# ay-lab/fithic

Measured on AMD Instinct MI355X. Metric: contact-pairs/sec through spline+p-value+BH pass (5 kb cis, whole node), higher is better.
Workload: dtype f64

## Files before the change

### fithic_amd/csrc/fhx_ctx.hpp

```cpp
#pragma once
#include <hip/hip_runtime.h>

#include <atomic>
#include <functional>
#include <chrono>
#include <thread>
#include <memory>
#include <sys/stat.h>
#include <unistd.h>
#include <deque>
#include <mutex>
#include <map>
#include <condition_variable>
#include <algorithm>
#include <climits>
#include <cstddef>
#include <cmath>
#include <cstdio>
#include <cstdlib>
#include <cstring>
#include <string>
#include <vector>

#include "../../include/fithic_mi355x.h"
#include "fhx_bdtrc.hpp"
#include "fhx_devmem.hpp"
#include "fhx_host.hpp"
#include "fhx_io_internal.hpp"
#include "fhx_scan.hpp"

namespace fhx {

__device__ __forceinline__ long long wave_sum_i64(long long v) {
#pragma unroll
    for (int off = 32; off > 0; off >>= 1) v += __shfl_down(v, off, 64);
    return v;
}
__device__ __forceinline__ int wave_max_i32(int v) {
#pragma unroll
    for (int off = 32; off > 0; off >>= 1) v = max(v, __shfl_down(v, off, 64));
    return v;
}

__device__ __forceinline__ unsigned int wave_incl_sum_u32(unsigned int v) {
    v += (unsigned int)__builtin_amdgcn_update_dpp(0, (int)v, 0x111, 0xf, 0xf, false);
    v += (unsigned int)__builtin_amdgcn_update_dpp(0, (int)v, 0x112, 0xf, 0xf, false);
    v += (unsigned int)__builtin_amdgcn_update_dpp(0, (int)v, 0x114, 0xf, 0xf, false);
    v += (unsigned int)__builtin_amdgcn_update_dpp(0, (int)v, 0x118, 0xf, 0xf, false);
    v += (unsigned int)__builtin_amdgcn_update_dpp(0, (int)v, 0x142, 0xa, 0xf, false);
    v += (unsigned int)__builtin_amdgcn_update_dpp(0, (int)v, 0x143, 0xc, 0xf, false);
    return v;
}

struct ChrGrid {
    int32_t base;
    int32_t off;
    int32_t nslots;
    int32_t pad;
};

struct K1Sums {
    long long inter_count, inter_sum, intra_all_count, intra_all_sum, in_range_count, in_range_sum, n_skipped;
    int max_count, pad;
};

struct K2Params {
    const int32_t* loc1;
    const int32_t* loc2;
    const int32_t* count;
    const double* slot_bias;
    bool no_bias;
    const double* prior_lut;
    int lut_len;
    dev::BinomTables intra, inter;
    double inter_chr_prob;
    double outlier_thres;
    int lo_idx, hi_idx;
    int mode;
    int64_t n;
    double* p;
    unsigned long long* top_hist;
    uint8_t* outlier;
    int nonfixed;
    const int32_t* slot_mid;
    const double* table_x;
    const double* table_y;
    int n_table;
    double min_x, max_x;
    long long dist_low, dist_up;
    double total_intra, total_inter;
};

constexpr int K2_THREADS = 256;

constexpr int K2_QUEUES = dev::BC_COUNT - 1;

struct QEntry {
    unsigned int row;
    int count;
    double prior;
};

constexpr int K2_MAX_SHARDS = 2048;

struct QSpan {
    QEntry* base;
    long long cap_s;
    int dir;
    int n_shards;
    const unsigned long long* count;
};
__device__ __forceinline__ QEntry* qentry(const QSpan& q, int shard, long long j) {
    return q.base + (long long)shard * q.cap_s + (long long)q.dir * j;
}

struct K2Queues {
    QSpan q[K2_QUEUES + 1];
    unsigned long long* count;
    unsigned int* heavy_hist;
};

constexpr int K2H_BUCKETS = 2048;
constexpr int K2H_BLOCKS = 1024;
__device__ __forceinline__ int k2h_bucket(int signed_count);

struct CutoffToHost {
    volatile unsigned long long* words = nullptr;
    unsigned long long ticket = 0;
    unsigned int* done = nullptr;
    unsigned long long* zero_me = nullptr;
};

constexpr int K3_DENSE_PERCENT = 35;
constexpr int K2_COUNTER_WORDS = 8;
constexpr int FDR_BUCKETS = 51;

struct DeviceWords {
    unsigned long long bh_kept;
    unsigned long long bh_cutoff;
    unsigned long long bh_below;
    unsigned long long array_kept;
    unsigned long long array_cutoff;
    unsigned long long sort_n;
    unsigned long long run_total;
    unsigned long long nf_keys;
    unsigned long long outliers_added;
    unsigned long long first_dup;
    unsigned long long memo_overflow;
    alignas(128) unsigned long long k2_redo;
    unsigned long long k2_next[K2_COUNTER_WORDS - 1];
    alignas(128) unsigned long long k3_dense;
    unsigned long long k3_sparse;
    alignas(128) unsigned long long fdr_buckets[FDR_BUCKETS];
};
static_assert(offsetof(DeviceWords, k2_next) == offsetof(DeviceWords, k2_redo) + sizeof(unsigned long long) &&
                  sizeof(DeviceWords::k2_next) == (K2_COUNTER_WORDS - 1) * sizeof(unsigned long long),
              "k2_closed zeroes K2_COUNTER_WORDS words starting at k2_redo");
static_assert(K2_COUNTER_WORDS >= 2 + K2_QUEUES, "k2_next holds k2h_heavy's word and one per class queue");
static_assert(sizeof(DeviceWords::fdr_buckets) == FDR_BUCKETS * sizeof(unsigned long long), "one word per FDR bucket");

constexpr int K2_CL_ITEMS = 4;
constexpr int K2_CL_TILE = K2_THREADS * K2_CL_ITEMS;

constexpr int K2_CLOSED = K2_QUEUES + 1;
constexpr int K2_CLOSED_LOCAL = K2_QUEUES + 2;
constexpr int K2_CLASSES = K2_QUEUES + 2;

constexpr int K2H_KCAP = 1023;
constexpr int K2H_GENERIC = 2 * K2H_KCAP;
constexpr int K2H_THREADS = 256;
constexpr int K2H_MAX_ROWS = 4;

constexpr int SORT_THREADS = 256;
constexpr int SORT_WAVES = SORT_THREADS / 64;
constexpr int SORT_ITEMS = 16;
constexpr int SORT_TILE = SORT_THREADS * SORT_ITEMS;
constexpr int CP_THREADS = 1024;
constexpr int CP_WAVES = CP_THREADS / 64;
constexpr int CP_ITEMS = 16;
constexpr int CP_TILE = CP_THREADS * CP_ITEMS;
constexpr int CP_STRIP = 2048;
constexpr int SORT_BLOCKS = 1024;
constexpr int RADIX_BITS = 11;
constexpr int RADIX = 1 << RADIX_BITS;
constexpr int SORT_PASSES = 6;
constexpr int SORT_BITS_LARGE = 8;

constexpr int TOP_SHIFT = 50;
constexpr int TOP_BINS = 8192;

__device__ __forceinline__ unsigned long long pvalue_key(double v) {
    unsigned long long bits = (unsigned long long)__double_as_longlong(v);
    if (bits == 0x8000000000000000ull) bits = 0ull;
    return bits;
}

constexpr unsigned long long KEY_ONE = 0x3FF0000000000000ull;
constexpr unsigned long long KEY_KEEP_ALL = 0x7FF0000000000001ull;

constexpr int SCAT_ITEMS = 8;
constexpr int BH_THREADS = 256;
constexpr int BH_ITEMS = 8;
constexpr int BH_TILE = BH_THREADS * BH_ITEMS;
constexpr int SEG_THREADS = 256;
constexpr int SEG_ITEMS = 16;
constexpr int SEG_TILE = SEG_THREADS * SEG_ITEMS;

}

using namespace fhx;

namespace fhx {
struct DistState;
struct K3Host;
}

struct FhxPinnedPair;
// ... 283 lines not shown
```

### fithic_amd/csrc/fhx_dist.inc

```
}

#include <dlfcn.h>
#include <rccl/rccl.h>
#include <chrono>

namespace fhx {
namespace ingest {
__global__ void ti_rebuild_rows(const int64_t* __restrict__ rows, int64_t n, int64_t n_loaded, const int32_t* __restrict__ loc1,
                                const int32_t* __restrict__ loc2, const int32_t* __restrict__ cnt, const int16_t* __restrict__ slot_chr,
                                const int32_t* __restrict__ slot_mid, const fhx::ChrGrid* __restrict__ grid, int32_t res,
                                int32_t* __restrict__ out, int* __restrict__ bad);
}

constexpr int DIST_MAX_SAMPLES = 8192;
constexpr unsigned long long DIST_SENTINEL = ~0ull;

__global__ void kd_pack_stats(const K1Sums* __restrict__ sums, const unsigned long long* __restrict__ hist_cc,
                              const unsigned long long* __restrict__ hist_np, int a, int w, int rank, int world,
                              long long* __restrict__ pack) {
    const int total = 8 + world + 2 * w;
    for (int i = blockIdx.x * blockDim.x + threadIdx.x; i < total; i += gridDim.x * blockDim.x) {
        long long v = 0;
        if (i < 7) {
            v = reinterpret_cast<const long long*>(sums)[i];
        } else if (i >= 8 && i < 8 + world) {
            v = (i - 8 == rank) ? (long long)sums->max_count : 0;
        } else if (i >= 8 + world && i < 8 + world + w) {
            v = (long long)hist_cc[a + (i - 8 - world)];
        } else if (i >= 8 + world + w) {
            v = (long long)hist_np[a + (i - 8 - world - w)];
        }
        pack[i] = v;
    }
}

__global__ void kd_samples(const unsigned long long* __restrict__ keys, const unsigned long long* __restrict__ n_ptr, int s,
                           unsigned long long* __restrict__ out) {
    const long long n = (long long)*n_ptr;
    for (int j = blockIdx.x * blockDim.x + threadIdx.x; j < s; j += gridDim.x * blockDim.x) {
        unsigned long long v = DIST_SENTINEL;
        if (n > 0) {
            long long at = ((long long)(j + 1) * n) / (s + 1);
            if (at > n - 1) at = n - 1;
            v = keys[at];
        }
        out[j] = v;
    }
}

__global__ __launch_bounds__(1024) void kd_splitters(const unsigned long long* __restrict__ samples, int total, int world,
                                                     unsigned long long* __restrict__ splitters) {
    __shared__ unsigned long long a[DIST_MAX_SAMPLES];
    __shared__ int n_valid;
    int N = 2;
    while (N < total) N <<= 1;
    for (int i = threadIdx.x; i < N; i += 1024) a[i] = i < total ? samples[i] : DIST_SENTINEL;
    if (threadIdx.x == 0) n_valid = 0;
    __syncthreads();
    for (int k = 2; k <= N; k <<= 1) {
        for (int j = k >> 1; j > 0; j >>= 1) {
            for (int i = threadIdx.x; i < N; i += 1024) {
                const int l = i ^ j;
                if (l > i) {
                    const unsigned long long x = a[i], y = a[l];
                    const bool up = (i & k) == 0;
                    if ((x > y) == up) {
                        a[i] = y;
                        a[l] = x;
                    }
                }
            }
            __syncthreads();
        }
    }
    int mine = 0;
    for (int i = threadIdx.x; i < N; i += 1024) mine += a[i] != DIST_SENTINEL;
    if (mine) atomicAdd(&n_valid, mine);
    __syncthreads();
    const int nv = n_valid;
    if ((int)threadIdx.x < world - 1) {
        unsigned long long v = DIST_SENTINEL;
        if (nv > 0) {
            long long pos = ((long long)(threadIdx.x + 1) * nv) / world;
            if (pos > nv - 1) pos = nv - 1;
            v = a[pos];
        }
        splitters[threadIdx.x] = v;
    }
    if (threadIdx.x == 0) splitters[world - 1] = (unsigned long long)nv;
}

__global__ void kd_cuts(const unsigned long long* __restrict__ keys, const unsigned long long* __restrict__ n_ptr,
                        const unsigned long long* __restrict__ splitters, int world, long long* __restrict__ counts) {
    __shared__ long long cut[65];
    const long long n = (long long)*n_ptr;
    const int r = threadIdx.x;
    if (r < world - 1) {
        const unsigned long long s = splitters[r];
        long long lo = 0, hi = n;
        if (splitters[world - 1] == 0ull) {
            lo = n;
        } else {
            while (lo < hi) {
                const long long mid = (lo + hi) >> 1;
                if (keys[mid] < s)
                    lo = mid + 1;
                else
                    hi = mid;
            }
        }
        cut[r + 1] = lo;
    }
    if (r == 0) {
        cut[0] = 0;
        cut[world] = n;
    }
    __syncthreads();
    if (r < world) counts[r] = cut[r + 1] - cut[r];
}

__global__ void kd_merge_runs(const unsigned long long* __restrict__ keys, const long long* __restrict__ off, int world,
                              unsigned long long* __restrict__ keys_out, unsigned int* __restrict__ arrival_out) {
    const long long m = off[world];
    for (long long i = (long long)blockIdx.x * blockDim.x + threadIdx.x; i < m; i += (long long)gridDim.x * blockDim.x) {
        int r = 0;
        while (r + 1 < world && i >= off[r + 1]) ++r;
        const unsigned long long k = keys[i];
        long long pos = i - off[r];
        for (int o = 0; o < world; ++o) {
            if (o == r) continue;
            long long lo = off[o], hi = off[o + 1];
            const bool take_equal = o < r;
            while (lo < hi) {
                const long long mid = (lo + hi) >> 1;
                const unsigned long long v = keys[mid];
                if (v < k || (take_equal && v == k))
                    lo = mid + 1;
                else
                    hi = mid;
            }
            pos += lo - off[o];
        }
        keys_out[pos] = k;
        arrival_out[pos] = (unsigned int)i;
    }
}

__global__ void kd_carry(const double* __restrict__ slice_max, int rank, double* __restrict__ carry) {
    double c = 0.0;
    for (int r = 0; r < rank; ++r) c = fmax(c, slice_max[r]);
    *carry = c;
}

struct RcclApi {
    void* lib = nullptr;
    ncclResult_t (*GetUniqueId)(ncclUniqueId*) = nullptr;
    ncclResult_t (*CommInitRank)(ncclComm_t*, int, ncclUniqueId, int) = nullptr;
    ncclResult_t (*CommDestroy)(ncclComm_t) = nullptr;
    ncclResult_t (*AllReduce)(const void*, void*, size_t, ncclDataType_t, ncclRedOp_t, ncclComm_t, hipStream_t) = nullptr;
    ncclResult_t (*AllGather)(const void*, void*, size_t, ncclDataType_t, ncclComm_t, hipStream_t) = nullptr;
    ncclResult_t (*Send)(const void*, size_t, ncclDataType_t, int, ncclComm_t, hipStream_t) = nullptr;
    ncclResult_t (*Recv)(void*, size_t, ncclDataType_t, int, ncclComm_t, hipStream_t) = nullptr;
    ncclResult_t (*GroupStart)() = nullptr;
    ncclResult_t (*GroupEnd)() = nullptr;
    const char* (*GetErrorString)(ncclResult_t) = nullptr;
    ncclResult_t (*GetVersion)(int*) = nullptr;
    std::string err;
};

static RcclApi* rccl_api() {
    static RcclApi api;
    static bool tried = false;
    if (tried) return api.lib ? &api : nullptr;
    tried = true;
    const char* env = getenv("FHX_RCCL_LIB");
// ... 723 lines not shown
```

### fithic_amd/csrc/fhx_k1.hip

```cpp
#include "fhx_ctx.hpp"
#include "fhx_k1key.hpp"

namespace fhx {

__global__ void k0_extent(const int32_t* __restrict__ chr, const int32_t* __restrict__ mid, int64_t n, int res,
                          int n_chr, int32_t* __restrict__ max_idx, int32_t* __restrict__ min_off,
                          int32_t* __restrict__ max_off, int32_t* __restrict__ bad) {
    const int64_t stride = (int64_t)gridDim.x * blockDim.x;
    for (int64_t i = (int64_t)blockIdx.x * blockDim.x + threadIdx.x; i < n; i += stride) {
        const int c = chr[i];
        const int m = mid[i];
        if (c < 0 || c >= n_chr || m < 0) {
            atomicOr(bad, 1);
            continue;
        }
        const int idx = m / res, off = m - idx * res;
        const bool full = __ballot(1) == ~0ull;
        const int c0 = __shfl(c, 0, 64);
        if (full && __ballot(c != c0) == 0ull) {
            int hi = idx, lo_off = off, hi_off = off;
            for (int s = 32; s >= 1; s >>= 1) {
                hi = max(hi, __shfl_xor(hi, s, 64));
                lo_off = min(lo_off, __shfl_xor(lo_off, s, 64));
                hi_off = max(hi_off, __shfl_xor(hi_off, s, 64));
            }
            if ((threadIdx.x & 63) == 0) {
                if (hi > max_idx[c]) atomicMax(&max_idx[c], hi);
                if (lo_off < min_off[c]) atomicMin(&min_off[c], lo_off);
                if (hi_off > max_off[c]) atomicMax(&max_off[c], hi_off);
            }
        } else {
            if (idx > max_idx[c]) atomicMax(&max_idx[c], idx);
            if (off < min_off[c]) atomicMin(&min_off[c], off);
            if (off > max_off[c]) atomicMax(&max_off[c], off);
        }
    }
}

__global__ void k0_slots(const int32_t* __restrict__ chr1, const int32_t* __restrict__ mid1,
                         const int32_t* __restrict__ chr2, const int32_t* __restrict__ mid2,
                         const int32_t* __restrict__ cnt, int64_t n, int res, const ChrGrid* __restrict__ grid,
                         int32_t* __restrict__ loc1, int32_t* __restrict__ loc2, int32_t* __restrict__ count,
                         uint32_t* __restrict__ key) {
    const int64_t stride = (int64_t)gridDim.x * blockDim.x;
    for (int64_t i = (int64_t)blockIdx.x * blockDim.x + threadIdx.x; i < n; i += stride) {
        const int c1 = chr1[i], c2 = chr2[i];
        const int s1 = grid[c1].base + mid1[i] / res;
        const int s2 = grid[c2].base + mid2[i] / res;
        const int l2 = (c1 == c2) ? s2 : ~s2;
        const int c = cnt[i];
        loc1[i] = s1;
        loc2[i] = l2;
        count[i] = c;
        key[i] = k1key::pack_row(s1, l2, c);
    }
}

constexpr int K1_THREADS = 512;
constexpr int K1_LDS_BINS = 6144;

constexpr int K1_WIDE_BINS = 24576;
constexpr int K1_WIDE_THREADS = 1024;

template <int THREADS, bool WIDE, bool KEYED>
__global__ __launch_bounds__(THREADS) void k1_classify_hist(
    const int32_t* __restrict__ loc1, const int32_t* __restrict__ loc2, const int32_t* __restrict__ count,
    const uint32_t* __restrict__ key, const uint8_t* __restrict__ skip, int64_t skip_limit, const long long* __restrict__ grow, int64_t n, int lo_idx,
    int hi_idx,
    unsigned long long* __restrict__ hist_sumcc, unsigned long long* __restrict__ hist_npairs,
    K1Sums* __restrict__ sums) {
    extern __shared__ __attribute__((aligned(16))) unsigned char smem[];
    constexpr int BINS = WIDE ? K1_WIDE_BINS : K1_LDS_BINS;
    unsigned long long* lds_cc = reinterpret_cast<unsigned long long*>(smem);
    unsigned int* lds_np = reinterpret_cast<unsigned int*>(smem + sizeof(unsigned long long) * K1_LDS_BINS);
    unsigned int* wide_sum = reinterpret_cast<unsigned int*>(smem);
    unsigned int* wide_cnt = reinterpret_cast<unsigned int*>(smem) + K1_WIDE_BINS;
    if (WIDE) {
        for (int i = threadIdx.x; i < BINS + BINS / 2; i += THREADS) wide_sum[i] = 0u;
    } else {
        for (int i = threadIdx.x; i < BINS; i += THREADS) {
            lds_cc[i] = 0ull;
            lds_np[i] = 0u;
        }
    }
    __syncthreads();

    long long inter_count = 0, inter_sum = 0, intra_cnt = 0, intra_sum = 0, rng_cnt = 0, rng_sum = 0, skipped = 0;
    int max_count = 0;

    auto one = [&](int l1, int l2, int c, int sk) {
        max_count = max(max_count, c);
        if (sk) {
            ++skipped;
            return;
        }
        if (l2 < 0) {
            ++inter_count;
            inter_sum += c;
            return;
        }
        ++intra_cnt;
        intra_sum += c;
        const int d = abs(l1 - l2);
        if (d >= lo_idx && d <= hi_idx) {
            ++rng_cnt;
            rng_sum += c;
            const int b = d - lo_idx;
            if (WIDE && b < BINS && c >= 0) {
                const unsigned int old = atomicAdd(&wide_sum[b], (unsigned int)c);
                if (old + (unsigned int)c < old) atomicAdd(&hist_sumcc[d], 1ull << 32);
                const int sh = (b & 1) * 16;
                const unsigned int was = (atomicAdd(&wide_cnt[b >> 1], 1u << sh) >> sh) & 0xFFFFu;
                if (was == 0x7FFFu) {
                    atomicSub(&wide_cnt[b >> 1], 0x8000u << sh);
                    atomicAdd(&hist_npairs[d], 32768ull);
                }
            } else if (!WIDE && b < BINS) {
                atomicAdd(&lds_cc[b], (unsigned long long)(long long)c);
                atomicAdd(&lds_np[b], 1u);
            } else {
                atomicAdd(&hist_sumcc[d], (unsigned long long)(long long)c);
                atomicAdd(&hist_npairs[d], 1ull);
            }
        }
    };

    auto keyed = [&](uint32_t k, int64_t row, int sk) {
        const k1key::Row r = k1key::unpack(k);
        if (r.escape)
            one(loc1[row], loc2[row], count[row], sk);
        else
            one(r.d, r.inter ? -1 : 0, r.count, sk);
    };

    const int64_t n4 = n >> 2;
    const int64_t stride = (int64_t)gridDim.x * blockDim.x;
    const int4* a4 = reinterpret_cast<const int4*>(loc1);
    const int4* b4 = reinterpret_cast<const int4*>(loc2);
    const int4* c4 = reinterpret_cast<const int4*>(count);
    const uint4* k4 = reinterpret_cast<const uint4*>(key);
    const uchar4* s4 = reinterpret_cast<const uchar4*>(skip);
    for (int64_t i = (int64_t)blockIdx.x * blockDim.x + threadIdx.x; i < n4; i += stride) {
        int4 a, b, c;
        uint4 k;
        if (KEYED) {
            k = k4[i];
        } else {
            a = a4[i];
            b = b4[i];
            c = c4[i];
        }
        uchar4 s = make_uchar4(0, 0, 0, 0);
        if (skip && grow) {
            s = s4[i];
            const int64_t r = i << 2;
            if (grow[r] > skip_limit) s.x = 0;
            if (grow[r + 1] > skip_limit) s.y = 0;
            if (grow[r + 2] > skip_limit) s.z = 0;
            if (grow[r + 3] > skip_limit) s.w = 0;
        } else if (skip && (i << 2) <= skip_limit) {
            s = s4[i];
            const int64_t r = i << 2;
            if (r + 1 > skip_limit) s.y = 0;
            if (r + 2 > skip_limit) s.z = 0;
            if (r + 3 > skip_limit) s.w = 0;
        }
        if (KEYED) {
            keyed(k.x, (i << 2), s.x);
            keyed(k.y, (i << 2) + 1, s.y);
            keyed(k.z, (i << 2) + 2, s.z);
            keyed(k.w, (i << 2) + 3, s.w);
        } else {
            one(a.x, b.x, c.x, s.x);
            one(a.y, b.y, c.y, s.y);
            one(a.z, b.z, c.z, s.z);
            one(a.w, b.w, c.w, s.w);
        }
    }
    if (blockIdx.x == 0 && threadIdx.x < (n & 3)) {
        const int64_t i = (n4 << 2) + threadIdx.x;
        const int sk = (skip && (grow ? grow[i] : i) <= skip_limit) ? skip[i] : 0;
        if (KEYED)
            keyed(key[i], i, sk);
        else
            one(loc1[i], loc2[i], count[i], sk);
    }

    __syncthreads();
    const int rot = (int)((blockIdx.x * 389u) % (unsigned)BINS);
    for (int k = threadIdx.x; k < BINS; k += THREADS) {
        int i = k + rot;
        if (i >= BINS) i -= BINS;
        if (WIDE) {
            const unsigned int sum = wide_sum[i], np = (wide_cnt[i >> 1] >> ((i & 1) * 16)) & 0xFFFFu;
            if (sum) atomicAdd(&hist_sumcc[lo_idx + i], (unsigned long long)sum);
            if (np) atomicAdd(&hist_npairs[lo_idx + i], (unsigned long long)np);
        } else {
            const unsigned int np = lds_np[i];
            if (np) {
                atomicAdd(&hist_sumcc[lo_idx + i], lds_cc[i]);
                atomicAdd(&hist_npairs[lo_idx + i], (unsigned long long)np);
            }
        }
    }
    inter_count = wave_sum_i64(inter_count);
    inter_sum = wave_sum_i64(inter_sum);
    intra_cnt = wave_sum_i64(intra_cnt);
    intra_sum = wave_sum_i64(intra_sum);
    rng_cnt = wave_sum_i64(rng_cnt);
    rng_sum = wave_sum_i64(rng_sum);
    skipped = wave_sum_i64(skipped);
    max_count = wave_max_i32(max_count);
    __syncthreads();
    long long* part = reinterpret_cast<long long*>(smem);
    constexpr int WAVES = THREADS / 64;
    const int w = threadIdx.x >> 6;
    if ((threadIdx.x & 63) == 0) {
        part[w * 8 + 0] = inter_count;
        part[w * 8 + 1] = inter_sum;
        part[w * 8 + 2] = intra_cnt;
        part[w * 8 + 3] = intra_sum;
        part[w * 8 + 4] = rng_cnt;
        part[w * 8 + 5] = rng_sum;
        part[w * 8 + 6] = skipped;
        part[w * 8 + 7] = max_count;
    }
    __syncthreads();
    if (threadIdx.x < 8) {
        long long v = part[threadIdx.x];
        for (int k = 1; k < WAVES; ++k) v = threadIdx.x == 7 ? max(v, part[k * 8 + 7]) : v + part[k * 8 + threadIdx.x];
        unsigned long long* dst = reinterpret_cast<unsigned long long*>(sums);
        if (threadIdx.x < 7) {
            if (v) atomicAdd(dst + threadIdx.x, (unsigned long long)v);
        } else {
            atomicMax(&sums->max_count, (int)v);
        }
    }
}

__global__ void k1_pack_window(const K1Sums* __restrict__ sums, const unsigned long long* __restrict__ hist_cc,
                               const unsigned long long* __restrict__ hist_np, int a, int w, long long* __restrict__ pack,
                               unsigned int* done, volatile unsigned long long* flag, unsigned long long ticket) {
    const int total = 8 + 2 * w;
    for (int i = blockIdx.x * blockDim.x + threadIdx.x; i < total; i += gridDim.x * blockDim.x) {
        long long v;
        if (i < 7)
            v = reinterpret_cast<const long long*>(sums)[i];
        else if (i == 7)
            v = (long long)sums->max_count;
        else if (i < 8 + w)
            v = (long long)hist_cc[a + (i - 8)];
        else
            v = (long long)hist_np[a + (i - 8 - w)];
        pack[i] = v;
    }
    if (flag) publish_ticket(done, flag, ticket);
}

__global__ void k1_prezero(unsigned long long* __restrict__ a, int64_t na, uint4* __restrict__ b, int64_t nb16, double* __restrict__ q,
                           int64_t n_q) {
    const int64_t stride = (int64_t)gridDim.x * blockDim.x;
    for (int64_t i = (int64_t)blockIdx.x * blockDim.x + threadIdx.x; i < nb16; i += stride) b[i] = make_uint4(0u, 0u, 0u, 0u);
    for (int64_t i = (int64_t)blockIdx.x * blockDim.x + threadIdx.x; i < na; i += stride) a[i] = 0ull;
    double2* q2 = reinterpret_cast<double2*>(q);
    const int64_t n2 = n_q >> 1;
    for (int64_t i = (int64_t)blockIdx.x * blockDim.x + threadIdx.x; i < n2; i += stride) q2[i] = make_double2(1.0, 1.0);
    if ((n_q & 1) && blockIdx.x == 0 && threadIdx.x == 0) q[n_q - 1] = 1.0;
}


__global__ void nf_locus_keys(const int32_t* __restrict__ c1, const int32_t* __restrict__ m1, const int32_t* __restrict__ c2,
                              const int32_t* __restrict__ m2, int64_t n, unsigned long long* __restrict__ keys,
                              unsigned int* __restrict__ vals, int* __restrict__ bad) {
    const int64_t stride = (int64_t)gridDim.x * blockDim.x;
    for (int64_t i = (int64_t)blockIdx.x * blockDim.x + threadIdx.x; i < n; i += stride) {
        if (c1[i] < 0 || c2[i] < 0 || m1[i] < 0 || m2[i] < 0) atomicOr(bad, 1);
        keys[i] = ((unsigned long long)(unsigned int)c1[i] << 32) | (unsigned int)m1[i];
        keys[n + i] = ((unsigned long long)(unsigned int)c2[i] << 32) | (unsigned int)m2[i];
        vals[i] = (unsigned int)i;
        vals[n + i] = (unsigned int)(n + i);
    }
}

__global__ __launch_bounds__(SEG_THREADS) void seg_count_heads(const unsigned long long* __restrict__ keys, int64_t n,
                                                               unsigned int* __restrict__ tile_heads) {
    __shared__ unsigned int cnt;
    if (threadIdx.x == 0) cnt = 0;
    __syncthreads();
    const int64_t base = (int64_t)blockIdx.x * SEG_TILE;
    unsigned int mine = 0;
    for (int r = 0; r < SEG_ITEMS; ++r) {
        const int64_t i = base + r * SEG_THREADS + threadIdx.x;
        if (i < n && (i == 0 || keys[i] != keys[i - 1])) ++mine;
    }
    mine = (unsigned int)wave_sum_i64((long long)mine);
    if ((threadIdx.x & 63) == 0 && mine) atomicAdd(&cnt, mine);
    __syncthreads();
    if (threadIdx.x == 0) tile_heads[blockIdx.x] = cnt;
}

__global__ __launch_bounds__(1024) void seg_scan_tiles(unsigned int* __restrict__ tile_heads, int64_t tiles,
                                                       unsigned long long* __restrict__ total) {
    __shared__ unsigned int part[1024];
    const int64_t per = (tiles + 1023) / 1024;
    const int64_t beg = (int64_t)threadIdx.x * per, end = min(tiles, beg + per);
    unsigned int sum = 0;
    for (int64_t t = beg; t < end; ++t) sum += tile_heads[t];
    part[threadIdx.x] = sum;
    __syncthreads();
    if (threadIdx.x == 0) {
        unsigned int acc = 0;
        for (int i = 0; i < 1024; ++i) {
            const unsigned int c = part[i];
            part[i] = acc;
            acc += c;
        }
        *total = acc;
    }
    __syncthreads();
    unsigned int run = part[threadIdx.x];
    for (int64_t t = beg; t < end; ++t) {
        const unsigned int c = tile_heads[t];
        tile_heads[t] = run;
        run += c;
    }
}

__global__ __launch_bounds__(SEG_THREADS) void seg_ids(const unsigned long long* __restrict__ keys, int64_t n,
                                                       const unsigned int* __restrict__ tile_base,
                                                       unsigned int* __restrict__ ids) {
    __shared__ unsigned int wtot[SEG_THREADS / 64];
    const int lane = threadIdx.x & 63, wave = threadIdx.x >> 6;
    const int64_t first = (int64_t)blockIdx.x * SEG_TILE + (int64_t)threadIdx.x * SEG_ITEMS;
    unsigned int heads = 0;
    unsigned int flag[SEG_ITEMS];
#pragma unroll
    for (int r = 0; r < SEG_ITEMS; ++r) {
        const int64_t i = first + r;
        flag[r] = (i < n && (i == 0 || keys[i] != keys[i - 1])) ? 1u : 0u;
        heads += flag[r];
    }
    unsigned int incl = heads;
#pragma unroll
    for (int off = 1; off < 64; off <<= 1) {
        const unsigned int o = __shfl_up(incl, off, 64);
        if (lane >= off) incl += o;
    }
    if (lane == 63) wtot[wave] = incl;
    __syncthreads();
    unsigned int before = tile_base[blockIdx.x] + incl - heads;
    for (int w = 0; w < wave; ++w) before += wtot[w];
#pragma unroll
    for (int r = 0; r < SEG_ITEMS; ++r) {
        const int64_t i = first + r;
        before += flag[r];
        if (i < n) ids[i] = before - 1;
    }
}

__global__ void nf_assign_slots(const unsigned long long* __restrict__ keys, const unsigned int* __restrict__ vals,
                                const unsigned int* __restrict__ ids, int64_t n2, int32_t* __restrict__ loc,
                                unsigned long long* __restrict__ slot_key) {
    const int64_t stride = (int64_t)gridDim.x * blockDim.x;
    for (int64_t i = (int64_t)blockIdx.x * blockDim.x + threadIdx.x; i < n2; i += stride) {
        loc[vals[i]] = (int32_t)ids[i];
        if (i == 0 || keys[i] != keys[i - 1]) slot_key[ids[i]] = keys[i];
    }
}

__global__ void nf_finish_rows(const int32_t* __restrict__ c1, const int32_t* __restrict__ c2, const int32_t* __restrict__ cnt,
                               const int32_t* __restrict__ loc, int64_t n, int32_t* __restrict__ loc1,
                               int32_t* __restrict__ loc2, int32_t* __restrict__ count) {
    const int64_t stride = (int64_t)gridDim.x * blockDim.x;
    for (int64_t i = (int64_t)blockIdx.x * blockDim.x + threadIdx.x; i < n; i += stride) {
        loc1[i] = loc[i];
        loc2[i] = (c1[i] == c2[i]) ? loc[n + i] : ~loc[n + i];
        count[i] = cnt[i];
    }
}

__global__ void nf_slot_tables(const unsigned long long* __restrict__ slot_key, int64_t n_slots, int32_t* __restrict__ slot_mid,
                               int16_t* __restrict__ slot_chr) {
    const int64_t stride = (int64_t)gridDim.x * blockDim.x;
    for (int64_t i = (int64_t)blockIdx.x * blockDim.x + threadIdx.x; i < n_slots; i += stride) {
        slot_mid[i] = (int32_t)(slot_key[i] & 0xFFFFFFFFull);
        slot_chr[i] = (int16_t)(slot_key[i] >> 32);
    }
}

__global__ __launch_bounds__(SORT_THREADS) void nf_k1_classify(
    const int32_t* __restrict__ loc1, const int32_t* __restrict__ loc2, const int32_t* __restrict__ count,
    const uint8_t* __restrict__ skip, int64_t skip_limit, const long long* __restrict__ grow, int64_t n,
    const int32_t* __restrict__ slot_mid, long long dist_low, long long dist_up, unsigned long long* __restrict__ keys,
    unsigned int* __restrict__ vals, unsigned long long* __restrict__ counter, K1Sums* __restrict__ sums) {
    __shared__ unsigned int wave_cnt[SORT_WAVES];
    __shared__ unsigned long long block_base;
    const int lane = threadIdx.x & 63, wave = threadIdx.x >> 6;
    const unsigned long long lane_lt = (1ull << lane) - 1ull;
// ... 653 lines not shown
```

### fithic_amd/csrc/fhx_k2.hip

```cpp
#include "fhx_ctx.hpp"

namespace fhx {

__device__ __forceinline__ double prior_by_search(const K2Params& P, long long dist) {
    double look = (double)dist;
    if (look < P.min_x) look = P.min_x;
    if (look > P.max_x) look = P.max_x;
    int lo = 0, hi = P.n_table;
    while (lo < hi) {
        const int mid = (lo + hi) >> 1;
        if (P.table_x[mid] < look)
            lo = mid + 1;
        else
            hi = mid;
    }
    return P.table_y[min(lo, P.n_table - 1)];
}

template <int NF = -1>
__device__ __forceinline__ bool row_prior(const K2Params& P, int l1, int l2, double& prior, bool& is_inter) {
    const bool inter = l2 < 0;
    const int s2 = inter ? ~l2 : l2;
    const double b1 = P.no_bias ? 1.0 : P.slot_bias[l1], b2 = P.no_bias ? 1.0 : P.slot_bias[s2];
    if ((b1 < 0 || b2 < 0) && !inter) return false;
// ... 343 lines not shown
    __device__ __forceinline__ int pair_of(unsigned int v) const {
        int lo = 0, hi = PAIRS;
#pragma unroll 1
        while (hi - lo > 1) {
            const int mid = (lo + hi) >> 1;
            if (prefix[mid] <= v)
                lo = mid;
            else
                hi = mid;
        }
        return lo;
    }
    struct Cursor {
        int pr;
        unsigned int base, end, c0;
    };
    __device__ __forceinline__ void load(Cursor& c) const {
        c.base = prefix[c.pr];
        c.end = prefix[c.pr + 1];
        c.c0 = (unsigned int)count[2 * c.pr];
    }
    __device__ __forceinline__ Cursor open(unsigned int v) const {
        Cursor c;
        c.pr = pair_of(v);
        load(c);
        return c;
    }
    __device__ __forceinline__ const QEntry* at(const QSpan& q, Cursor& c, unsigned int v) const {
        if (v >= c.end) {
            do ++c.pr;
            while (v >= prefix[c.pr + 1]);
            load(c);
        }
        const unsigned int u = v - c.base;
        return u < c.c0 ? qentry(q, 2 * c.pr, (long long)u) : qentry(q, 2 * c.pr + 1, (long long)(u - c.c0));
    }
};
constexpr int K2_WAVES = K2_THREADS / 64;

template <int CLS, bool SMALL_N>
__global__ __launch_bounds__(K2_THREADS) void k2_queue(K2Params P, QSpan q) {
    __shared__ unsigned int hist_lds[K2_HIST_BINS];
    __shared__ unsigned int prefix_lds[QDense::PAIRS + 1], wave_tot[K2_WAVES];
    constexpr bool LEAN = CLS == dev::BC_PSERIES;
    __shared__ double rtab[LEAN ? dev::kPsTabJ : 1];
    if (LEAN) dev::div_table_build<false>(rtab, dev::kPsTabJ);
    FusedHist H;
    H.init(hist_lds, P.top_hist);
    QDense D;
    D.build(q, prefix_lds, wave_tot);
    const unsigned long long total = D.total();
    const unsigned int lane = threadIdx.x & 63;
    const unsigned long long n_waves = (unsigned long long)gridDim.x * K2_WAVES;
    const unsigned long long share = ((total + n_waves - 1) / n_waves + 63ull) & ~63ull;
    const unsigned long long begin = ((unsigned long long)blockIdx.x * K2_WAVES + (threadIdx.x >> 6)) * share;
    const unsigned long long end = min(total, begin + share);
    QDense::Cursor cur{0, 0u, 0u, 0u};
    if (begin + lane < end) cur = D.open((unsigned int)(begin + lane));
#pragma unroll 1
    for (unsigned long long v = begin + lane; v < end; v += 64) {
        const QEntry e = *D.at(q, cur, (unsigned int)v);
        const bool is_inter = e.count < 0;
        const int c = is_inter ? -e.count : e.count;
        const double pv = dev::bdtrc_count_class<CLS, SMALL_N, LEAN>(c, is_inter ? P.inter : P.intra, e.prior, rtab);
        store_p<false>(P.p + e.row, pv);
        H.add(pv);
    }
    H.flush(P.top_hist);
}

constexpr int K2_SORT_TILE = 1024;
constexpr int K2_SORT_BUCKETS = 32;
template <int CLS, bool SMALL_N, int WPE>
__global__ __launch_bounds__(K2_THREADS) __attribute__((amdgpu_waves_per_eu(WPE))) void k2_queue_by_count(K2Params P, QSpan q,
                                                                                                         unsigned int* next_tile) {
    static_assert(K2_SORT_TILE == 4 * K2_THREADS, "four entries per thread");
    __shared__ QEntry tile[K2_SORT_TILE];
    __shared__ unsigned int bucket_cnt[K2_SORT_BUCKETS], bucket_off[K2_SORT_BUCKETS];
    __shared__ unsigned int hist_lds[K2_HIST_BINS];
    __shared__ unsigned int prefix_lds[QDense::PAIRS + 1], wave_tot[K2_WAVES], tile_lds;
    __shared__ double ytab[dev::kCfTabJ];
    dev::div_table_build<true>(ytab, dev::kCfTabJ);
    FusedHist H;
    H.init(hist_lds, P.top_hist);
    QDense D;
    D.build(q, prefix_lds, wave_tot);
    const unsigned int total = D.total();
    const unsigned int share = (total + gridDim.x - 1) / gridDim.x;
    const unsigned int rounds = max(1u, (share + K2_SORT_TILE - 1) / K2_SORT_TILE);
    const unsigned int tile_n = max(min((unsigned int)K2_SORT_TILE, ((share + rounds - 1) / rounds + 63u) & ~63u), 64u);
    const unsigned int tiles = (total + tile_n - 1) / tile_n;
    unsigned int mine = blockIdx.x;
    for (;;) {
        if (threadIdx.x < K2_SORT_BUCKETS) bucket_cnt[threadIdx.x] = 0;
        if (threadIdx.x == 0) tile_lds = mine;
        __syncthreads();
        const unsigned int t = tile_lds;
        if (t >= tiles) break;
        if (threadIdx.x == 0) mine = gridDim.x + atomicAdd(next_tile, 1u);
        const unsigned int v0 = t * tile_n;
        const int m = (int)min(tile_n, total - v0);
        QEntry e[4];
        int bucket[4];
        unsigned int slot[4];
        QDense::Cursor cur{0, 0u, 0u, 0u};
        if ((int)threadIdx.x < m) cur = D.open(v0 + threadIdx.x);
#pragma unroll
        for (int r = 0; r < 4; ++r) {
            const int idx = r * K2_THREADS + (int)threadIdx.x;
            bucket[r] = -1;
            if (idx < m) {
                e[r] = *D.at(q, cur, v0 + idx);
                const int c = e[r].count < 0 ? -e[r].count : e[r].count;
                bucket[r] = c < K2_SORT_BUCKETS - 1 ? c : K2_SORT_BUCKETS - 1;
                slot[r] = atomicAdd(&bucket_cnt[bucket[r]], 1u);
            }
        }
        __syncthreads();
        if (threadIdx.x < K2_SORT_BUCKETS) {
            unsigned int off = 0;
            for (int b = 0; b < (int)threadIdx.x; ++b) off += bucket_cnt[b];
            bucket_off[threadIdx.x] = off;
        }
        __syncthreads();
#pragma unroll
        for (int r = 0; r < 4; ++r)
            if (bucket[r] >= 0) tile[bucket_off[bucket[r]] + slot[r]] = e[r];
        __syncthreads();
#pragma unroll 1
        for (int r = 0; r < 4; ++r) {
            const int idx = r * K2_THREADS + threadIdx.x;
            if (idx < m) {
                const QEntry x = tile[idx];
                const bool is_inter = x.count < 0;
                const int c = is_inter ? -x.count : x.count;
                const double pv = dev::bdtrc_count_class<CLS, SMALL_N, true>(c, is_inter ? P.inter : P.intra, x.prior, ytab);
                store_p<false>(P.p + x.row, pv);
                H.add(pv);
            }
        }
        __syncthreads();
    }
    H.flush(P.top_hist);
}



__device__ __forceinline__ int k2h_bucket(int signed_count) {
    const bool inter = signed_count < 0;
    const int c = inter ? -signed_count : signed_count;
    return c < K2H_KCAP ? (inter ? K2H_KCAP + c : c) : K2H_GENERIC;
}

__global__ __launch_bounds__(K2H_THREADS) void k2h_scatter(QSpan q, const unsigned int* __restrict__ block_hist,
                                                           const unsigned int* __restrict__ off, QEntry* __restrict__ out) {
    __shared__ unsigned int cursor[K2H_BUCKETS];
    for (int d = threadIdx.x; d < K2H_BUCKETS; d += K2H_THREADS) cursor[d] = off[d] + block_hist[(size_t)d * K2H_BLOCKS + blockIdx.x];
    __syncthreads();
    for (int sh = blockIdx.x; sh < q.n_shards; sh += K2H_BLOCKS) {
        const long long n = (long long)q.count[sh];
        for (long long i = threadIdx.x; i < n; i += K2H_THREADS) {
            const QEntry e = *qentry(q, sh, i);
            out[atomicAdd(&cursor[k2h_bucket(e.count)], 1u)] = e;
        }
    }
}

static_assert(dev::kCfIters <= 1024, "one thread per table row");
__device__ __forceinline__ void k2h_table_row(const unsigned int* __restrict__ digit_total, double n_intra, double n_inter,
                                              dev::CfRow* __restrict__ tab) {
    const int b = blockIdx.x;
    if (digit_total[b] == 0 || (int)threadIdx.x >= dev::kCfIters) return;
    const bool inter = b >= K2H_KCAP;
    tab[(size_t)b * dev::kCfIters + threadIdx.x] = dev::cf_swapped_row(inter ? n_inter : n_intra, inter ? b - K2H_KCAP : b, (int)threadIdx.x);
}
__global__ __launch_bounds__(1024) void k2h_offsets_and_tables(const unsigned int* __restrict__ digit_total, unsigned int* __restrict__ off,
                                                               unsigned int granule, double n_intra, double n_inter, dev::CfRow* __restrict__ tab) {
    if (blockIdx.x < K2H_GENERIC) {
        k2h_table_row(digit_total, n_intra, n_inter, tab);
        return;
    }
    __shared__ unsigned int part[1024];
    const unsigned int g1 = granule - 1u;
    const unsigned int a = (digit_total[2 * threadIdx.x] + g1) / granule * granule, b = (digit_total[2 * threadIdx.x + 1] + g1) / granule * granule;
    const int lane = threadIdx.x & 63, wave = threadIdx.x >> 6;
    const unsigned int incl = wave_incl_sum_u32(a + b);
    if (lane == 63) part[wave] = incl;
    __syncthreads();
    unsigned int excl = incl - (a + b);
    for (int w = 0; w < wave; ++w) excl += part[w];
    if (threadIdx.x == 1023) off[K2H_BUCKETS] = excl + a + b;
    off[2 * threadIdx.x] = excl;
    off[2 * threadIdx.x + 1] = excl + a;
}


struct K2HeavyParams {
    dev::BinomTables intra, inter;
    double* p;
    unsigned long long* top_hist;
};
__device__ unsigned long long g_k2h_clk[4];

template <int R, int WPE, bool SMALL_N>
__global__ __launch_bounds__(K2H_THREADS) __attribute__((amdgpu_waves_per_eu(WPE, WPE))) void k2h_heavy(
    K2HeavyParams P, const QEntry* __restrict__ sorted, const unsigned int* __restrict__ off,
    const unsigned int* __restrict__ digit_total, const dev::CfRow* __restrict__ tab, QEntry* __restrict__ redo,
    unsigned long long* __restrict__ n_redo, unsigned int* __restrict__ next_task) {
    static_assert(R >= 1 && R <= K2H_MAX_ROWS, "the sorted queue is padded for at most K2H_MAX_ROWS rows per lane");
    __shared__ unsigned int hist_lds[K2_HIST_BINS];
    FusedHist H;
    H.init(hist_lds, P.top_hist);
    const int wave = __builtin_amdgcn_readfirstlane((int)(threadIdx.x >> 6));
    const int lane = threadIdx.x & 63;
    constexpr unsigned int TASK = 64u * R;
    const unsigned int n_tasks = off[K2H_GENERIC] / TASK;
    const unsigned int n_waves = gridDim.x * (K2H_THREADS / 64);
    if (blockIdx.x == 0 && threadIdx.x == 0) {
        g_k2h_clk[0] = __builtin_amdgcn_s_memtime();
        g_k2h_clk[1] = __builtin_amdgcn_s_memrealtime();
    }
    for (unsigned int task = blockIdx.x * (K2H_THREADS / 64) + wave; task < n_tasks;) {
        const unsigned int first = task * TASK;
        int lo = 0, hi = K2H_GENERIC;
        while (hi - lo > 1) {
            const int mid = (lo + hi) >> 1;
            if (off[mid] <= first)
                lo = mid;
            else
                hi = mid;
        }
        const int b = __builtin_amdgcn_readfirstlane(lo);
        const unsigned int live = off[b] + digit_total[b];
        const bool is_inter = b >= K2H_KCAP;
        const int c = is_inter ? b - K2H_KCAP : b;
        const dev::BinomTables& T = is_inter ? P.inter : P.intra;
        const double fk = (double)c - 1.0;
        const double aa = fk + 1.0, bb = T.n - fk;
        const unsigned int last = live > first ? live - 1u : first;
        QEntry e[R];
        bool have[R], irregular[R];
        double w1[R], cf[R];
#pragma unroll
        for (int r = 0; r < R; ++r) {
            const unsigned int j = first + (unsigned int)r * 64u + (unsigned int)lane;
            have[r] = j < live;
            e[r] = sorted[have[r] ? j : last];
            w1[r] = 1.0 - e[r].prior;
            irregular[r] = !dev::cf_swapped_regular(bb, aa, w1[r]);
        }
        const dev::CfRowConstPtr rows = (dev::CfRowConstPtr)(uintptr_t)(tab + (size_t)b * dev::kCfIters);
        dev::cf_swapped_uniform<R>(rows, w1, irregular, cf);
#pragma unroll
        for (int r = 0; r < R; ++r) {
            w1[r] = 1.0 - e[r].prior;
            double pv = 0.0;
            const bool mine = have[r] && !irregular[r];
            if (have[r]) {
                if (__builtin_expect(irregular[r], 0))
                    redo[atomicAdd(n_redo, 1ull)] = e[r];
                else {
                    pv = dev::incbet_finish<SMALL_N>(bb, aa, w1[r], e[r].prior, cf[r], 1, T.lbeta[c], (SMALL_N && T.small_n) ? T.inv_beta[c] : 0.0);
                    store_p<true>(P.p + e[r].row, pv);
                }
            }
            H.add_wave_min(pv, mine);
        }
        unsigned int next = 0;
        if (lane == 0) next = atomicAdd(next_task, 1u);
        task = n_waves + (unsigned int)__builtin_amdgcn_readfirstlane((int)next);
    }
    if (blockIdx.x == 0 && threadIdx.x == 0) {
        g_k2h_clk[2] = __builtin_amdgcn_s_memtime();
        g_k2h_clk[3] = __builtin_amdgcn_s_memrealtime();
    }
    H.flush(P.top_hist);
}

__global__ __launch_bounds__(K2_THREADS) void k2h_generic(K2Params P, const QEntry* __restrict__ sorted,
                                                          const unsigned int* __restrict__ off,
                                                          const unsigned int* __restrict__ digit_total,
                                                          const QEntry* __restrict__ redo,
                                                          const unsigned long long* __restrict__ n_redo) {
    const QEntry* base = sorted + off[K2H_GENERIC];
    const int64_t n_generic = (int64_t)digit_total[K2H_GENERIC];
    const int64_t n = n_generic + (int64_t)*n_redo;
    __shared__ unsigned int hist_lds[K2_HIST_BINS];
    FusedHist H;
    H.init(hist_lds, P.top_hist);
    const int64_t stride = (int64_t)gridDim.x * blockDim.x;
    for (int64_t j = (int64_t)blockIdx.x * blockDim.x + threadIdx.x; j < n; j += stride) {
        const QEntry e = j < n_generic ? base[j] : redo[j - n_generic];
        const bool is_inter = e.count < 0;
        const int c = is_inter ? -e.count : e.count;
        const double pv = dev::bdtrc_count_class<dev::BC_CF_SWAPPED>(c, is_inter ? P.inter : P.intra, e.prior);
        store_p<true>(P.p + e.row, pv);
        H.add(pv);
    }
    H.flush(P.top_hist);
}


__global__ void k_debug_classify(double n_total, const int32_t* __restrict__ count, const double* __restrict__ prior, int64_t n,
                                 int32_t* __restrict__ by_table, int32_t* __restrict__ by_arith, double* __restrict__ thr5) {
    const int64_t i = (int64_t)blockIdx.x * blockDim.x + threadIdx.x;
    if (i >= n) return;
    const dev::ClsRow r = dev::cls_row(n_total, count[i]);
    by_table[i] = dev::cls_is_trivial(count[i], n_total, prior[i]) ? (int)dev::BC_TRIVIAL : dev::cls_lookup(r, prior[i]);
    by_arith[i] = dev::bdtrc_class(count[i], n_total, prior[i]);
    if (thr5) {
        thr5[5 * i] = r.tA;
        thr5[5 * i + 1] = r.tB;
        thr5[5 * i + 2] = r.tC;
        thr5[5 * i + 3] = r.tD;
        thr5[5 * i + 4] = r.tE;
    }
// ... 882 lines not shown
```

Baseline: 14.27 billion.

## Batch loads in k1 classify and k2h scatter, derive range sums from histogram

The k1 classify loop now issues four strided vector loads per thread before processing them, so more memory requests are in flight. It also drops the per-row in-range count and sum accumulation, recomputing those totals in the pack kernels by reducing the histogram window. k2h_scatter likewise loads four queue entries before performing the LDS-atomic scatter. The trade-off is higher register pressure, and the histogram-derived sums could differ from the originals if some in-range rows fall outside the histogram bins or have negative counts.

```diff
diff --git a/fithic_amd/csrc/fhx_ctx.hpp b/fithic_amd/csrc/fhx_ctx.hpp
--- a/fithic_amd/csrc/fhx_ctx.hpp
+++ b/fithic_amd/csrc/fhx_ctx.hpp
@@ -63,6 +63,47 @@
     long long inter_count, inter_sum, intra_all_count, intra_all_sum, in_range_count, in_range_sum, n_skipped;
     int max_count, pad;
 };
+
+__device__ __forceinline__ void k1_window_sums(const unsigned long long* __restrict__ hist_cc, const unsigned long long* __restrict__ hist_np,
+                                               int a, int w, long long* rows, long long* sum) {
+    __shared__ unsigned long long part[2][16];
+    unsigned long long np = 0ull, cc = 0ull;
+    const int T = (int)blockDim.x;
+    for (int j0 = (int)threadIdx.x; j0 < w; j0 += 4 * T) {
+        unsigned long long x[4], y[4];
+#pragma unroll
+        for (int u = 0; u < 4; ++u) {
+            const int j = min(j0 + u * T, w - 1);
+            x[u] = hist_np[a + j];
+            y[u] = hist_cc[a + j];
+        }
+#pragma unroll
+        for (int u = 0; u < 4; ++u) {
+            if (j0 + u * T < w) {
+                np += x[u];
+                cc += y[u];
+            }
+        }
+    }
+#pragma unroll
+    for (int off = 32; off > 0; off >>= 1) {
+        np += __shfl_down(np, off, 64);
+        cc += __shfl_down(cc, off, 64);
+    }
+    if ((threadIdx.x & 63) == 0) {
+        part[0][threadIdx.x >> 6] = np;
+        part[1][threadIdx.x >> 6] = cc;
+    }
+    __syncthreads();
+    if (threadIdx.x == 0) {
+        for (int k = 1; k < (T >> 6); ++k) {
+            np += part[0][k];
+            cc += part[1][k];
+        }
+        *rows = (long long)np;
+        *sum = (long long)cc;
+    }
+}
 
 struct K2Params {
     const int32_t* loc1;
diff --git a/fithic_amd/csrc/fhx_dist.inc b/fithic_amd/csrc/fhx_dist.inc
--- a/fithic_amd/csrc/fhx_dist.inc
+++ b/fithic_amd/csrc/fhx_dist.inc
@@ -19,8 +19,17 @@
                               const unsigned long long* __restrict__ hist_np, int a, int w, int rank, int world,
                               long long* __restrict__ pack) {
     const int total = 8 + world + 2 * w;
+    if (blockIdx.x == 0) {
+        long long rows = 0, sum = 0;
+        k1_window_sums(hist_cc, hist_np, a, w, &rows, &sum);
+        if (threadIdx.x == 0) {
+            pack[4] = rows;
+            pack[5] = sum;
+        }
+    }
     for (int i = blockIdx.x * blockDim.x + threadIdx.x; i < total; i += gridDim.x * blockDim.x) {
         long long v = 0;
+        if (i == 4 || i == 5) continue;
         if (i < 7) {
             v = reinterpret_cast<const long long*>(sums)[i];
         } else if (i >= 8 && i < 8 + world) {
diff --git a/fithic_amd/csrc/fhx_k1.hip b/fithic_amd/csrc/fhx_k1.hip
--- a/fithic_amd/csrc/fhx_k1.hip
+++ b/fithic_amd/csrc/fhx_k1.hip
@@ -61,6 +61,7 @@
 
 constexpr int K1_WIDE_BINS = 24576;
 constexpr int K1_WIDE_THREADS = 1024;
+constexpr int K1_INFLIGHT = 4;
 
 template <int THREADS, bool WIDE, bool KEYED>
 __global__ __launch_bounds__(THREADS) void k1_classify_hist(
@@ -85,7 +86,7 @@
     }
     __syncthreads();
 
-    long long inter_count = 0, inter_sum = 0, intra_cnt = 0, intra_sum = 0, rng_cnt = 0, rng_sum = 0, skipped = 0;
+    long long inter_count = 0, inter_sum = 0, intra_cnt = 0, intra_sum = 0, skipped = 0;
     int max_count = 0;
 
     auto one = [&](int l1, int l2, int c, int sk) {
@@ -103,8 +104,6 @@
         intra_sum += c;
         const int d = abs(l1 - l2);
         if (d >= lo_idx && d <= hi_idx) {
-            ++rng_cnt;
-            rng_sum += c;
             const int b = d - lo_idx;
             if (WIDE && b < BINS && c >= 0) {
                 const unsigned int old = atomicAdd(&wide_sum[b], (unsigned int)c);
@@ -140,41 +139,58 @@
     const int4* c4 = reinterpret_cast<const int4*>(count);
     const uint4* k4 = reinterpret_cast<const uint4*>(key);
     const uchar4* s4 = reinterpret_cast<const uchar4*>(skip);
-    for (int64_t i = (int64_t)blockIdx.x * blockDim.x + threadIdx.x; i < n4; i += stride) {
-        int4 a, b, c;
-        uint4 k;
-        if (KEYED) {
-            k = k4[i];
-        } else {
-            a = a4[i];
-            b = b4[i];
-            c = c4[i];
-        }
-        uchar4 s = make_uchar4(0, 0, 0, 0);
-        if (skip && grow) {
-            s = s4[i];
+    const longlong2* g2 = reinterpret_cast<const longlong2*>(grow);
+    constexpr int U = K1_INFLIGHT;
+    for (int64_t i0 = (int64_t)blockIdx.x * blockDim.x + threadIdx.x; i0 < n4; i0 += U * stride) {
+        int4 a[U], b[U], c[U];
+        uint4 k[U];
+        uchar4 s[U];
+        longlong2 g[U][2];
+#pragma unroll
+        for (int u = 0; u < U; ++u) {
+            const int64_t i = min(i0 + u * stride, n4 - 1);
+            if (KEYED) {
+                k[u] = k4[i];
+            } else {
+                a[u] = a4[i];
+                b[u] = b4[i];
+                c[u] = c4[i];
+            }
+            s[u] = make_uchar4(0, 0, 0, 0);
+            if (skip && grow) {
+                s[u] = s4[i];
+                g[u][0] = g2[2 * i];
+                g[u][1] = g2[2 * i + 1];
+            } else if (skip && (i << 2) <= skip_limit) {
+                s[u] = s4[i];
+            }
+        }
+#pragma unroll
+        for (int u = 0; u < U; ++u) {
+            const int64_t i = i0 + u * stride;
+            if (i >= n4) break;
             const int64_t r = i << 2;
-            if (grow[r] > skip_limit) s.x = 0;
-            if (grow[r + 1] > skip_limit) s.y = 0;
-            if (grow[r + 2] > skip_limit) s.z = 0;
-            if (grow[r + 3] > skip_limit) s.w = 0;
-        } else if (skip && (i << 2) <= skip_limit) {
-            s = s4[i];
-            const int64_t r = i << 2;
-            if (r + 1 > skip_limit) s.y = 0;
-            if (r + 2 > skip_limit) s.z = 0;
-            if (r + 3 > skip_limit) s.w = 0;
-        }
-        if (KEYED) {
-            keyed(k.x, (i << 2), s.x);
-            keyed(k.y, (i << 2) + 1, s.y);
-            keyed(k.z, (i << 2) + 2, s.z);
-            keyed(k.w, (i << 2) + 3, s.w);
-        } else {
-            one(a.x, b.x, c.x, s.x);
-            one(a.y, b.y, c.y, s.y);
-            one(a.z, b.z, c.z, s.z);
-            one(a.w, b.w, c.w, s.w);
+            if (skip && grow) {
+                if (g[u][0].x > skip_limit) s[u].x = 0;
+                if (g[u][0].y > skip_limit) s[u].y = 0;
+                if (g[u][1].x > skip_limit) s[u].z = 0;
+                if (g[u][1].y > skip_limit) s[u].w = 0;
+            } else if (skip && r <= skip_limit) {
+                if (r + 1 > skip_limit) s[u].y = 0;
+                if (r + 2 > skip_limit) s[u].z = 0;
+                if (r + 3 > skip_limit) s[u].w = 0;
+            }
+            if (KEYED) {
+                keyed(k[u].x, r, s[u].x);
+                keyed(k[u].y, r + 1, s[u].y);
+                keyed(k[u].z, r + 2, s[u].z);
+                keyed(k[u].w, r + 3, s[u].w);
+            } else {
+                one(a[u].x, b[u].x, c[u].x, s[u].x);
+                one(a[u].y, b[u].y, c[u].y, s[u].y);
+                one(a[u].z, b[u].z, c[u].z, s[u].z);
+                one(a[u].w, b[u].w, c[u].w, s[u].w);
+            }
         }
     }
     if (blockIdx.x == 0 && threadIdx.x < (n & 3)) {
@@ -207,8 +223,6 @@
     inter_sum = wave_sum_i64(inter_sum);
     intra_cnt = wave_sum_i64(intra_cnt);
     intra_sum = wave_sum_i64(intra_sum);
-    rng_cnt = wave_sum_i64(rng_cnt);
-    rng_sum = wave_sum_i64(rng_sum);
     skipped = wave_sum_i64(skipped);
     max_count = wave_max_i32(max_count);
     __syncthreads();
@@ -220,8 +234,8 @@
         part[w * 8 + 1] = inter_sum;
         part[w * 8 + 2] = intra_cnt;
         part[w * 8 + 3] = intra_sum;
-        part[w * 8 + 4] = rng_cnt;
-        part[w * 8 + 5] = rng_sum;
+        part[w * 8 + 4] = 0;
+        part[w * 8 + 5] = 0;
         part[w * 8 + 6] = skipped;
         part[w * 8 + 7] = max_count;
     }
@@ -242,8 +256,17 @@
                                const unsigned long long* __restrict__ hist_np, int a, int w, long long* __restrict__ pack,
                                unsigned int* done, volatile unsigned long long* flag, unsigned long long ticket) {
     const int total = 8 + 2 * w;
+    if (blockIdx.x == 0) {
+        long long rows = 0, sum = 0;
+        k1_window_sums(hist_cc, hist_np, a, w, &rows, &sum);
+        if (threadIdx.x == 0) {
+            pack[4] = rows;
+            pack[5] = sum;
+        }
+    }
     for (int i = blockIdx.x * blockDim.x + threadIdx.x; i < total; i += gridDim.x * blockDim.x) {
         long long v;
+        if (i == 4 || i == 5) continue;
         if (i < 7)
             v = reinterpret_cast<const long long*>(sums)[i];
         else if (i == 7)
diff --git a/fithic_amd/csrc/fhx_k2.hip b/fithic_amd/csrc/fhx_k2.hip
--- a/fithic_amd/csrc/fhx_k2.hip
+++ b/fithic_amd/csrc/fhx_k2.hip
@@ -519,16 +519,29 @@
     return c < K2H_KCAP ? (inter ? K2H_KCAP + c : c) : K2H_GENERIC;
 }
 
+constexpr int K2H_SCATTER_INFLIGHT = 4;
 __global__ __launch_bounds__(K2H_THREADS) void k2h_scatter(QSpan q, const unsigned int* __restrict__ block_hist,
                                                            const unsigned int* __restrict__ off, QEntry* __restrict__ out) {
     __shared__ unsigned int cursor[K2H_BUCKETS];
     for (int d = threadIdx.x; d < K2H_BUCKETS; d += K2H_THREADS) cursor[d] = off[d] + block_hist[(size_t)d * K2H_BLOCKS + blockIdx.x];
     __syncthreads();
+    constexpr int U = K2H_SCATTER_INFLIGHT;
     for (int sh = blockIdx.x; sh < q.n_shards; sh += K2H_BLOCKS) {
         const long long n = (long long)q.count[sh];
-        for (long long i = threadIdx.x; i < n; i += K2H_THREADS) {
-            const QEntry e = *qentry(q, sh, i);
-            out[atomicAdd(&cursor[k2h_bucket(e.count)], 1u)] = e;
+        for (long long i0 = threadIdx.x; i0 < n; i0 += U * K2H_THREADS) {
+            if (i0 + (U - 1) * K2H_THREADS < n) {
+                QEntry e[U];
+#pragma unroll
+                for (int u = 0; u < U; ++u) e[u] = *qentry(q, sh, i0 + u * K2H_THREADS);
+                __builtin_amdgcn_sched_barrier(0);
+#pragma unroll
+                for (int u = 0; u < U; ++u) out[atomicAdd(&cursor[k2h_bucket(e[u].count)], 1u)] = e[u];
+            } else {
+                for (long long i = i0; i < n; i += K2H_THREADS) {
+                    const QEntry e = *qentry(q, sh, i);
+                    out[atomicAdd(&cursor[k2h_bucket(e.count)], 1u)] = e;
+                }
+            }
         }
     }
 }
```

Result: no change. 14.32 billion (median of 6 runs) (+0.4%).
